# ZeningLin/PEneo

Measured on AMD Instinct MI355X. Metric: docs/sec fwd+bwd, LayoutLMv3-base seq512 L128, higher is better.
Workload: dtype bf16; 1 GPU; LayoutLMv3-base PEneo, synthetic RFUND-shaped batch seq512/128 lines, 8 docs/GPU, train mode (dropout 0.1), fwd+loss+bwd; docs_per_gpu=8, seq_len=512, lines=128, parallelism=dp1

## Files before the change

include/peneo_hip.h:

```cpp
#ifndef PENEO_HIP_H
#define PENEO_HIP_H

#include <stddef.h>
#include <stdint.h>

#ifdef __cplusplus
extern "C" {
#endif

#define PENEO_OK 0
#define PENEO_ERR_INVALID (-1)
#define PENEO_ERR_LAUNCH (-2)

#define PENEO_F32 0
#define PENEO_BF16 1

#define PENEO_ACT_NONE 0
#define PENEO_ACT_GELU 1
#define PENEO_ACT_SILU 2

#define PENEO_MAX_HEADS 8

typedef void* peneo_stream_t;

// ... 308 lines not shown
  int32_t step_offset; int32_t reserved;
} peneo_adamw_tensor;
int peneo_adamw_chunk_elems(void);
int peneo_adamw_step(const peneo_adamw_tensor* table_dev, const int32_t* chunk_tensor_dev, const int32_t* chunk_index_dev,
                     int n_chunks, float beta1, float beta2, float eps, int step, peneo_stream_t stream);
int peneo_grad_sqnorm_slots(void);
int peneo_grad_sqnorm(const peneo_adamw_tensor* table_dev, const int32_t* chunk_tensor_dev, const int32_t* chunk_index_dev,
                      int n_chunks, double* sqnorm_dev, peneo_stream_t stream);
int peneo_adamw_step_clip(const peneo_adamw_tensor* table_dev, const int32_t* chunk_tensor_dev, const int32_t* chunk_index_dev,
                          int n_chunks, float beta1, float beta2, float eps, int step, const double* sqnorm_dev,
                          float max_grad_norm, peneo_stream_t stream);
typedef struct peneo_adamw_emit { void* dst; int32_t tensor; int32_t dtype; } peneo_adamw_emit;
int peneo_adamw_step_emit(const peneo_adamw_tensor* table_dev, const int32_t* chunk_tensor_dev, const int32_t* chunk_index_dev,
                          int n_chunks, float beta1, float beta2, float eps, int step, const double* sqnorm_dev,
                          float max_grad_norm, const peneo_adamw_emit* emits_dev, const int32_t* emit_first_dev,
                          peneo_stream_t stream);

typedef struct peneo_encoder_layer {
  const void* Wqkv; const float* bqkv; const void* Wo; const float* bo; const float* g1; const float* b1;
  const void* Wi; const float* bi; const void* Wo2; const float* bo2; const float* g2; const float* b2;
  const void* bias; int64_t bias_ld; const float* key_bias; const uint32_t* drop_words;
  const void* x; void* qkv; void* att; float* lse; void* h1; float* m1; float* r1; void* a; void* zi; void* inter; void* h2;
  float* m2; float* r2;
  int32_t B, T, H, nh, I, reserved;
  float eps, attn_scale, p_hidden, p_attn;
  uint32_t seed_o, seed_o2;
} peneo_encoder_layer;
typedef struct peneo_encoder_layer_grads {
  const void* d_out; void* d_x;
  void* d_h2; void* d_dense2; void* d_zi; void* d_a; void* d_h1; void* d_dense1; void* d_att; void* dqkv; float* delta; void* ds_out;
  float* dwqkv; float* dbqkv; float* dwo; float* dbo; float* dg1; float* db1; float* dwi; float* dbi; float* dwo2; float* dbo2;
  float* dg2; float* db2;
} peneo_encoder_layer_grads;
size_t peneo_struct_bytes(int which);
size_t peneo_encoder_layer_workspace_bytes(int rows, int H, int I, int which);
int peneo_encoder_layer_fwd(const peneo_encoder_layer* layer, void* out, void* workspace, size_t workspace_bytes,
                            peneo_stream_t stream);
int peneo_encoder_layer_fwd_packed(const peneo_encoder_layer* layer, const int32_t* lens, const int32_t* cu_rows, int rows, void* out,
                                   void* workspace, size_t workspace_bytes, peneo_stream_t stream);
typedef struct peneo_encoder_layer_mxfp8 {
  const void* Wqkv_q; const void* Wqkv_s; const void* Wo_q; const void* Wo_s;
  const void* Wi_q; const void* Wi_s; const void* Wo2_q; const void* Wo2_s;
  void* x_q; void* x_s; void* att_q; void* att_s; void* a_q; void* a_s; void* inter_q; void* inter_s;
  void* out_q; void* out_s;
  int32_t x_prequantized, reserved;
} peneo_encoder_layer_mxfp8;
int peneo_encoder_layer_mxfp8_supported(int rows, int H, int I);
// ... 3 lines not shown
                            size_t ws_main_bytes, void* ws_side, size_t ws_side_bytes, peneo_stream_t stream,
                            peneo_stream_t side_stream);

int peneo_spots_to_tags(const int32_t* spots_bijt, int n_spots, int B, int N, int64_t* tags, int32_t* status,
                        peneo_stream_t stream);
int peneo_spots_compact(const float* logits, int64_t P, int C, int N, int32_t* spots_ijt, float* scores,
                        int32_t* count, int max_spots, peneo_stream_t stream);

typedef struct peneo_spots_batch_desc {
  int num_maps;
  int classes[PENEO_MAX_HEADS];
  const void* maps[PENEO_MAX_HEADS];
} peneo_spots_batch_desc;
size_t peneo_spots_compact_batch_workspace_bytes(int num_maps, int B, int N);
int peneo_spots_compact_batch(const peneo_spots_batch_desc* desc, int B, int N, void* records, int32_t* counts,
                              int max_spots, void* workspace, size_t workspace_bytes, peneo_stream_t stream);

void peneo_gemm_set_big_mode(int mode);
int peneo_gemm_big_mode(void);
void peneo_gemm_set_nn384_mode(int mode);
int peneo_gemm_nn384_mode(void);
uint64_t peneo_gemm_nn384_launches(void);
int peneo_gemm_nn384_shape_ok(int M, int N, int K);
void peneo_gemm_set_sk_mode(int mode);
void peneo_gemm_sk_set_prof(void* stamps);
void peneo_gemm_sk_set_max_groups(int n);

void peneo_set_deterministic(int mode);
int peneo_deterministic(void);
uint64_t peneo_order_dependent_launches(void);
int64_t peneo_pair_bwd_workspace_rows(int B, int N);
int64_t peneo_pair_dz_fused_workspace_rows(int64_t npairs);
size_t peneo_relpos_bwd_workspace_bytes(int nh, int bins1, int bins2);
int peneo_relpos_bias_bwd_layers_ws(const void* ds, int L, int64_t layer_stride, const uint8_t* bk1_t, const uint8_t* bkx_t,
                                    const uint8_t* bky_t, float* dw1, int bins1, float* dwx, float* dwy, int bins2, float scale,
                                    int B, int nh, int T, int Tp, void* workspace, size_t workspace_bytes, peneo_stream_t stream);
int peneo_relpos_bias_bwd_ws(const float* g, int64_t ldg, const uint8_t* bk1, const uint8_t* bkx, const uint8_t* bky, float* dw1,
                             int bins1, float* dwx, float* dwy, int bins2, float scale, int B, int nh, int T, void* workspace,
                             size_t workspace_bytes, peneo_stream_t stream);
size_t peneo_grad_sqnorm_workspace_bytes(int n_chunks);
int peneo_grad_sqnorm_ws(const peneo_adamw_tensor* table_dev, const int32_t* chunk_tensor_dev, const int32_t* chunk_index_dev,
                         int n_chunks, double* sqnorm_dev, void* workspace, size_t workspace_bytes, peneo_stream_t stream);

#ifdef __cplusplus
}
#endif
// ... 2 lines not shown
```

peneo_amd/csrc/common.h:

```cpp
#pragma once
#include <hip/hip_runtime.h>
#include <stdint.h>
#include <cstdlib>

#include "../../include/peneo_hip.h"

namespace peneo {

typedef unsigned short bf16_t;
typedef __attribute__((ext_vector_type(8))) __bf16 bf16x8_t;
typedef __attribute__((ext_vector_type(16))) float f32x16_t;
typedef __attribute__((ext_vector_type(4))) float f32x4_t;

constexpr int kWave = 64;

void set_error(const char* fmt, ...);
int check_launch(const char* what);

int det_mode();
int order_dependent(const char* entry_point);
#define PENEO_ORDER_DEPENDENT(entry_point)                        \
  do {                                                            \
    const int od_rc_ = ::peneo::order_dependent(entry_point);     \
    if (od_rc_ != PENEO_OK) return od_rc_;                        \
  } while (0)

inline int dynamic_lds_error(const char* entry_point, size_t bytes) {
  set_error("%s: cannot raise dynamic LDS to %zu bytes", entry_point, bytes);
  return PENEO_ERR_LAUNCH;
}
template <typename KernelT>
inline int raise_dynamic_lds(KernelT kernel, size_t bytes, const char* entry_point) {
  const void* fn = reinterpret_cast<const void*>(kernel);
  if (hipFuncSetAttribute(fn, hipFuncAttributeMaxDynamicSharedMemorySize, (int)bytes) == hipSuccess) return PENEO_OK;
  return dynamic_lds_error(entry_point, bytes);
}
inline bool env_switch_on(const char* name) { const char* e = getenv(name); return !e || atoi(e) != 0; }

#define PENEO_REQUIRE(cond, ...)                \
  do {                                          \
    if (!(cond)) {                              \
      ::peneo::set_error(__VA_ARGS__);          \
      return PENEO_ERR_INVALID;                 \
    }                                           \
  } while (0)

__device__ __forceinline__ float bf16_to_f32(bf16_t v) { return __uint_as_float(((uint32_t)v) << 16); }

// ... 273 lines not shown
```

peneo_amd/csrc/gemm.hip:

```cpp
#include <cstdlib>
#include "common.h"
#include "gemm_common.h"

namespace peneo {

__device__ __forceinline__ int lds_off(int row, int slot) { return row * ROWB + ((slot ^ ((row >> 1) & 7)) << 4); }

template <typename T> struct Stage { uint4 v[4]; };

template <typename T>
__device__ __forceinline__ uint4 guarded_vec_load(const T* base, int64_t ld, int r, int c, int rmax, int cmax) {
  constexpr int VEC = Elem<T>::kVec;
  uint4 z = make_uint4(0, 0, 0, 0);
  if (r >= rmax || c >= cmax) return z;
  const T* p = base + (int64_t)r * ld + c;
  if (c + VEC <= cmax && ((reinterpret_cast<uintptr_t>(p) & 15) == 0)) return *reinterpret_cast<const uint4*>(p);
  float f[VEC];
#pragma unroll
  for (int e = 0; e < VEC; ++e) f[e] = (c + e < cmax) ? Elem<T>::load(p + e) : 0.f;
  return pack16<T>(f);
}

template <typename T>
__device__ __forceinline__ void load_kmajor(Stage<T>& s, const T* base, int64_t ld, int r0, int k0, int rmax, int kmax,
// ... 672 lines not shown
  if constexpr (CS) {
    if (cs_on && (lane & 31) == 0) {
#pragma unroll
      for (int r = 0; r < 16; ++r) {
        const int m = m0 + wm * 64 + wn * 32 + acc_row(r, lane);
        if (m < p.M) atomicAdd(p.ep.a_colsum + m, accb[r]);
      }
    }
  }
  tile_epilogue<DZ>(p, acc, smem, m0, n0, tid, lane, wm, wn, dzpre, zsplit);
}

template <bool AK, bool BK, bool CS = false, bool DZ = false>
__global__ __launch_bounds__(256, 2) void gemm_dma_pipe_kernel(GemmParams p) {
  extern __shared__ __attribute__((aligned(16))) char smem[];
  const int gx = gridDim.x, gxy = gx * gridDim.y, total = gxy * gridDim.z;
  const int lin = (blockIdx.z * gridDim.y + blockIdx.y) * gx + blockIdx.x;
  const int q8 = total >> 3, r8 = total & 7, xcd = lin & 7, slot = lin >> 3;
  const int tile3 = xcd * q8 + min(xcd, r8) + slot;
  const int zsplit = tile3 / gxy, tile = tile3 - zsplit * gxy;
  gemm_dma_pipe_body<AK, BK, CS, DZ>(p, smem, (tile / gx) * GB, (tile % gx) * GB, zsplit, tile % gx, gx);
}

constexpr int GEMM_GROUP_MAX = 4;
struct GemmGroup {
  GemmParams p[GEMM_GROUP_MAX];
  int first_tile[GEMM_GROUP_MAX + 1];
  int gx[GEMM_GROUP_MAX];
  int n;
};
template <bool AK, bool BK>
__global__ __launch_bounds__(256, 2) void gemm_dma_pipe_group_kernel(GemmGroup g) {
  extern __shared__ __attribute__((aligned(16))) char smem[];
  const int total = gridDim.x, lin = blockIdx.x;
  const int q8 = total >> 3, r8 = total & 7, xcd = lin & 7, slot = lin >> 3;
  const int tile3 = xcd * q8 + min(xcd, r8) + slot;
  int i = 0;
#pragma unroll
  for (int k = 1; k < GEMM_GROUP_MAX; ++k)
    if (k < g.n && tile3 >= g.first_tile[k]) i = k;
  const int tile = tile3 - g.first_tile[i], gx = g.gx[i];
  gemm_dma_pipe_body<AK, BK>(g.p[i], smem, (tile / gx) * GB, (tile % gx) * GB, 0);
}

__global__ void splitk_reduce_kernel(GemmParams p) {
  int64_t idx = (int64_t)blockIdx.x * blockDim.x + threadIdx.x;
  int64_t total = (int64_t)p.M * p.N;
// ... 59 lines not shown
    return check_launch("peneo_gemm");
  }
  if (ak && bk) hipLaunchKernelGGL((gemm_dma_pipe_kernel<true, true>), grid, dim3(256), shmem, st, p);
  else if (ak && !bk) hipLaunchKernelGGL((gemm_dma_pipe_kernel<true, false>), grid, dim3(256), shmem, st, p);
  else if (!ak && bk) hipLaunchKernelGGL((gemm_dma_pipe_kernel<false, true>), grid, dim3(256), shmem, st, p);
  else if (p.ep.a_colsum) hipLaunchKernelGGL((gemm_dma_pipe_kernel<false, false, true>), grid, dim3(256), shmem, st, p);
  else hipLaunchKernelGGL((gemm_dma_pipe_kernel<false, false>), grid, dim3(256), shmem, st, p);
  return check_launch("peneo_gemm");
}


}

using namespace peneo;

extern "C" size_t peneo_gemm_workspace_bytes(int M, int N, int K, int split_k) {
  const size_t partials = split_k > 1 ? (size_t)split_k * (size_t)M * (size_t)N * sizeof(float) : 0;
  const size_t stream_k = gemm_sk_workspace_bytes(M, N, K);
  return partials > stream_k ? partials : stream_k;
}

extern "C" int peneo_gemm_group(int dtype, int a_kmajor, int b_kmajor, int c_dtype, const peneo_gemm_problem* problems, int n,
                                peneo_stream_t stream) {
  PENEO_REQUIRE(dtype == PENEO_BF16, "peneo_gemm_group: bf16 operands only");
  PENEO_REQUIRE(c_dtype == PENEO_F32 || c_dtype == PENEO_BF16, "peneo_gemm_group: bad c_dtype %d", c_dtype);
  PENEO_REQUIRE(problems && n >= 1 && n <= GEMM_GROUP_MAX, "peneo_gemm_group: 1..%d problems (got %d)", GEMM_GROUP_MAX, n);
  auto dma_ok = [](const void* ptr, int64_t ld, bool kmajor, int rows, int k) {
    return (reinterpret_cast<uintptr_t>(ptr) & 15) == 0 && (ld % 8) == 0 && ((kmajor ? k : rows) % 8) == 0 && rows >= 8;
  };
  GemmGroup g;
  g.n = n;
  int tiles = 0;
  for (int i = 0; i < GEMM_GROUP_MAX; ++i) {
    const peneo_gemm_problem& q = problems[i < n ? i : n - 1];
    if (i < n) {
      PENEO_REQUIRE(q.M > 0 && q.N > 0 && q.K > 0 && q.A && q.B && q.C, "peneo_gemm_group: problem %d is empty or has a null operand", i);
      PENEO_REQUIRE(q.lda >= (a_kmajor ? q.K : q.M) && q.ldb >= (b_kmajor ? q.K : q.N) && q.ldc >= q.N,
                    "peneo_gemm_group: problem %d: leading dim too small", i);
      PENEO_REQUIRE(dma_ok(q.A, q.lda, a_kmajor != 0, q.M, q.K) && dma_ok(q.B, q.ldb, b_kmajor != 0, q.N, q.K),
                    "peneo_gemm_group: problem %d: operands must be 16-byte aligned with extents in whole 16-byte chunks", i);
      PENEO_REQUIRE(!q.accumulate || c_dtype == PENEO_F32, "peneo_gemm_group: accumulate needs an fp32 C");
    }
    GemmParams& p = g.p[i];
    p.A = q.A; p.B = q.B; p.C = q.C; p.lda = q.lda; p.ldb = q.ldb; p.ldc = q.ldc; p.M = q.M; p.N = q.N; p.K = q.K;
    p.c_dtype = c_dtype;
    peneo_gemm_epilogue z = {};
    p.ep = (i < n && q.ep) ? *q.ep : z;
    if (i < n && q.ep) {
      PENEO_REQUIRE(!q.ep->pair_dz && !q.ep->a_colsum, "peneo_gemm_group: problem %d: pair_dz / a_colsum are not available in a group", i);
      PENEO_REQUIRE(q.ep->drop_p >= 0.f && q.ep->drop_p < 1.f, "peneo_gemm_group: problem %d: drop_p out of range", i);
      PENEO_REQUIRE(!q.ep->accumulate || c_dtype == PENEO_F32, "peneo_gemm_group: accumulate needs an fp32 C");
    }
    if (p.ep.alpha == 0.f) p.ep.alpha = 1.f;
    if (q.accumulate) p.ep.accumulate = 1;
    p.split_k = 1; p.ws = nullptr; p.kt_per_split = (q.K + 63) / 64; p.dz_on = 0; p.dz_ws = nullptr;
    peneo_pair_dz_args za = {};
    p.dz = za;
    g.first_tile[i] = tiles;
    g.gx[i] = (q.N + GB - 1) / GB;
    if (i < n) tiles += g.gx[i] * ((q.M + GB - 1) / GB);
  }
  g.first_tile[GEMM_GROUP_MAX] = tiles;
  for (int i = n; i < GEMM_GROUP_MAX; ++i) g.first_tile[i] = tiles;
  const int shmem = 2 * 2 * TILE_BYTES;
  hipStream_t st = reinterpret_cast<hipStream_t>(stream);
  const bool ak = a_kmajor != 0, bk = b_kmajor != 0;
#define PENEO_GROUP_LAUNCH(AK_, BK_)                                                                                         \
  {                                                                                                                          \
    static std::atomic<uint64_t> lds_devices{0};                                                                             \
    if (!allow_dynamic_lds(reinterpret_cast<const void*>(gemm_dma_pipe_group_kernel<AK_, BK_>), shmem, lds_devices))         \
      return dynamic_lds_error("peneo_gemm_group", shmem);                                                                   \
    hipLaunchKernelGGL((gemm_dma_pipe_group_kernel<AK_, BK_>), dim3((unsigned)tiles), dim3(256), shmem, st, g);              \
  }
  if (ak && bk) PENEO_GROUP_LAUNCH(true, true)
  else if (ak && !bk) PENEO_GROUP_LAUNCH(true, false)
  else if (!ak && bk) PENEO_GROUP_LAUNCH(false, true)
  else PENEO_GROUP_LAUNCH(false, false)
#undef PENEO_GROUP_LAUNCH
  return check_launch("peneo_gemm_group");
}

extern "C" int peneo_gemm(int dtype, int a_kmajor, int b_kmajor, int M, int N, int K, const void* A, int64_t lda,
                          const void* B, int64_t ldb, void* C, int64_t ldc, int c_dtype,
                          const peneo_gemm_epilogue* ep, int split_k, void* workspace, size_t workspace_bytes,
                          peneo_stream_t stream) {
  PENEO_REQUIRE(dtype == PENEO_F32 || dtype == PENEO_BF16, "peneo_gemm: bad dtype %d", dtype);
  PENEO_REQUIRE(c_dtype == PENEO_F32 || c_dtype == PENEO_BF16, "peneo_gemm: bad c_dtype %d", c_dtype);
  PENEO_REQUIRE(M > 0 && N > 0 && K > 0, "peneo_gemm: empty problem %dx%dx%d", M, N, K);
  PENEO_REQUIRE(A && B && C, "peneo_gemm: null operand");
// ... 86 lines not shown
```

peneo_amd/csrc/gemm_big.hip:

```cpp
#include <cstdlib>
#include <type_traits>
#include "common.h"
#include "gemm_common.h"

namespace peneo {

typedef short bg_s16x4 __attribute__((ext_vector_type(4)));

template <bool BK_, int WGM_, int WGN_, int FM_, int FN_, int NSTAGE_, bool AK_ = true>
struct BigCfg {
  static constexpr bool AK = AK_, BK = BK_;
  static constexpr int WGM = WGM_, WGN = WGN_, FM = FM_, FN = FN_, NSTAGE = NSTAGE_;
  static constexpr int BM = WGM * FM * 32, BN = WGN * FN * 32;
  static constexpr int A_BYTES = BM * 128, B_BYTES = BN * 128, STAGE = A_BYTES + B_BYTES;
  static constexpr int APW = BM / 64, BPW = BN / 64, PPW = APW + BPW;
  static constexpr int LDS_BYTES = NSTAGE * STAGE;
  static constexpr int EP_LD = FN * 32 + 4;
  static_assert(WGM * WGN == 8, "eight waves");
  static_assert(BM % 64 == 0 && BN % 64 == 0, "pieces of 8 rows are dealt to 8 waves");
  static_assert(8 * 32 * EP_LD * 4 <= LDS_BYTES, "epilogue patches fit in the dead ring");
  static_assert(LDS_BYTES <= 160 * 1024, "LDS");
};

template <typename C, bool PART = false>
__global__ __launch_bounds__(512) void gemm_big_kernel(GemmParams p, int tiles_n) {
  extern __shared__ __attribute__((aligned(16))) char smem[];
  constexpr int FM = C::FM, FN = C::FN, NSTAGE = C::NSTAGE;
  const int tid = threadIdx.x, lane = tid & 63, half = lane >> 5;
  const int wave = __builtin_amdgcn_readfirstlane(tid >> 6);
  const int wm = wave / C::WGN, wn = wave % C::WGN;

  const int total = gridDim.x, lin = blockIdx.x;
  const int q8 = total >> 3, r8 = total & 7, xcd = lin & 7, slot = lin >> 3;
  int tile = xcd * q8 + min(xcd, r8) + slot;
  int zsplit = 0, kt0 = 0, ktiles = p.K / 64;
  if constexpr (PART) {
    const int tiles = total / p.split_k;
    zsplit = tile / tiles;
    tile -= zsplit * tiles;
    kt0 = zsplit * p.kt_per_split;
    ktiles = min(ktiles, kt0 + p.kt_per_split) - kt0;
  }
  const int m0 = (tile / tiles_n) * C::BM, n0 = (tile % tiles_n) * C::BN;

  const bf16_t* A = reinterpret_cast<const bf16_t*>(p.A);
  const bf16_t* B = reinterpret_cast<const bf16_t*>(p.B);

  uint32_t offA[C::APW], offB[C::BPW];
#pragma unroll
  for (int u = 0; u < C::APW; ++u) {
    const int g = wave + 8 * u;
    if constexpr (C::AK) {
      const int row = g * 8 + (lane >> 3);
      const int sg = (lane & 7) ^ ((row >> 1) & 7);
      offA[u] = (uint32_t)(((int64_t)(min(m0 + row, p.M - 1) - m0) * p.lda + sg * 8) * 2);
    } else {
      constexpr int MQ = C::BM / 64;
      const int kb = g / MQ, mq = g % MQ, kr = lane >> 3;
      const int cg = (lane & 7) ^ (((kr >> 1) & 1) << 2);
      offA[u] = (uint32_t)(((int64_t)(kb * 8 + kr) * p.lda + (min(m0 + mq * 64 + cg * 8, p.M - 8) - m0)) * 2);
    }
  }
#pragma unroll
  for (int u = 0; u < C::BPW; ++u) {
    const int g = wave + 8 * u;
    if constexpr (C::BK) {
// ... 116 lines not shown
    const bool more = t + NSTAGE - 1 < ktiles;
    dbase = __builtin_amdgcn_readfirstlane(lds0 + ((t + NSTAGE - 1) % NSTAGE) * C::STAGE + wave * 1024);
    const char* st = smem + (t % NSTAGE) * C::STAGE;
    uint4 fa0[FM], fb0[FN], fa1[FM], fb1[FN];
    load_a(st, 0, fa0); load_b(st, 0, fb0);
    if (more) issue_group(std::integral_constant<int, 0>{});
    load_a(st, 1, fa1); load_b(st, 1, fb1);
    __builtin_amdgcn_sched_barrier(0);
    mma(fa0, fb0);
    __builtin_amdgcn_sched_barrier(0);
    if (more) issue_group(std::integral_constant<int, 1>{});
    load_a(st, 2, fa0); load_b(st, 2, fb0);
    __builtin_amdgcn_sched_barrier(0);
    mma(fa1, fb1);
    __builtin_amdgcn_sched_barrier(0);
    if (more) issue_group(std::integral_constant<int, 2>{});
    load_a(st, 3, fa1); load_b(st, 3, fb1);
    __builtin_amdgcn_sched_barrier(0);
    mma(fa0, fb0);
    __builtin_amdgcn_sched_barrier(0);
    if (more) issue_group(std::integral_constant<int, 3>{});
    mma(fa1, fb1);
  }
  __syncthreads();

  float* patch = reinterpret_cast<float*>(smem) + wave * (32 * C::EP_LD);
  constexpr int CG = FN * 32 / 8;
  constexpr int RPP = 64 / CG;
  constexpr int NPASS = (32 + RPP - 1) / RPP;
  const int cgi = lane % CG, rli = lane / CG;
  auto block = [&](auto ic) {
    constexpr int i = decltype(ic)::value;
#pragma unroll
    for (int j = 0; j < FN; ++j)
#pragma unroll
      for (int r = 0; r < 16; ++r) patch[acc_row(r, lane) * C::EP_LD + j * 32 + acc_col(lane)] = acc[i][j][r];
    __builtin_amdgcn_wave_barrier();
    const int mb = m0 + (wm * FM + i) * 32, nb = n0 + wn * FN * 32 + cgi * 8;
#pragma unroll 1
    for (int pass = 0; pass < NPASS; ++pass) {
      const int rl = pass * RPP + rli;
      if (rli < RPP && rl < 32 && mb + rl < p.M && nb + 8 <= p.N) {
        float v[8];
        const float4 x0 = *reinterpret_cast<const float4*>(patch + rl * C::EP_LD + cgi * 8);
        const float4 x1 = *reinterpret_cast<const float4*>(patch + rl * C::EP_LD + cgi * 8 + 4);
        v[0] = x0.x; v[1] = x0.y; v[2] = x0.z; v[3] = x0.w; v[4] = x1.x; v[5] = x1.y; v[6] = x1.z; v[7] = x1.w;
        if constexpr (PART) {
          float4* q = reinterpret_cast<float4*>(p.ws + ((int64_t)zsplit * p.M + (mb + rl)) * p.N + nb);
          q[0] = x0; q[1] = x1;
        } else {
          epilogue_store8(p, mb + rl, nb, v);
        }
      }
    }
    __builtin_amdgcn_wave_barrier();
  };
  block(std::integral_constant<int, 0>{});
  if constexpr (FM > 1) block(std::integral_constant<int, 1>{});
  if constexpr (FM > 2) block(std::integral_constant<int, 2>{});
  if constexpr (FM > 3) block(std::integral_constant<int, 3>{});
  static_assert(FM <= 4, "row blocks");
}

template <typename C, bool PART = false>
static int launch_big(const GemmParams& p, hipStream_t st) {
  const int tm = (p.M + C::BM - 1) / C::BM, tn = (p.N + C::BN - 1) / C::BN;
  static std::atomic<uint64_t> lds_devices{0};
  if (!allow_dynamic_lds(reinterpret_cast<const void*>(gemm_big_kernel<C, PART>), C::LDS_BYTES, lds_devices))
    return dynamic_lds_error("peneo_gemm", C::LDS_BYTES);
  const int wgs = tm * tn * (PART ? p.split_k : 1);
  hipLaunchKernelGGL((gemm_big_kernel<C, PART>), dim3((unsigned)wgs), dim3(512), C::LDS_BYTES, st, p, tn);
  const int rc = check_launch("peneo_gemm (big tiles)");
  return rc == PENEO_OK ? 1 : rc;
}

template <bool BK> using Big256 = BigCfg<BK, 2, 4, 4, 2, 2>;
template <bool BK> using Big384 = BigCfg<BK, 4, 2, 3, 3, 2>;
template <bool BK> using Big128 = BigCfg<BK, 4, 2, 2, 2, 3>;

static double big_cost(int M, int N, int bm, int bn, double per_round) {
  const int tiles = ((M + bm - 1) / bm) * ((N + bn - 1) / bn);
  return ((tiles + 255) / 256) * per_round;
}
static double small_cost(int M, int N) {
// ... 40 lines not shown
    if (pick == 128) return launch_big<Big128<true>>(p, st);
    return launch_big<Big256<true>>(p, st);
  }
  if (pick == 384) return launch_big<Big384<false>>(p, st);
  if (pick == 128) return launch_big<Big128<false>>(p, st);
  return launch_big<Big256<false>>(p, st);
}

using BigNN384 = BigCfg<false, 4, 2, 3, 3, 2, false>;
constexpr int NN_MIN_K = 65536;

static int g_nn_mode = -1;

static std::atomic<uint64_t> g_nn_launches{0};

static int nn_mode() {
  if (g_nn_mode < 0) { const char* e = getenv("PENEO_GEMM_NN384"); g_nn_mode = e ? atoi(e) : 1; }
  return big_mode() == 0 ? 0 : g_nn_mode;
}

static bool nn_shape_ok(int M, int N, int K) {
  const int mode = nn_mode();
  if (mode == 0 || M <= 0 || N <= 0 || K <= 0) return false;
  if (M % BigNN384::BM != 0 || N % BigNN384::BN != 0 || K % 64 != 0) return false;
  return mode != 1 || K >= NN_MIN_K;
}

int launch_gemm_big_nn(const GemmParams& p, hipStream_t st) {
  if (!nn_shape_ok(p.M, p.N, p.K)) return 0;
  const peneo_gemm_epilogue& e = p.ep;
  if (p.c_dtype != PENEO_F32 || p.dz_on || e.bias || e.preact || e.grad_src || e.residual || e.a_colsum || e.act != PENEO_ACT_NONE ||
      e.drop_p != 0.f || e.alpha != 1.f)
    return 0;
  if ((reinterpret_cast<uintptr_t>(p.A) | reinterpret_cast<uintptr_t>(p.B) | reinterpret_cast<uintptr_t>(p.C)) & 15) return 0;
  if (p.lda % 8 != 0 || p.ldb % 8 != 0 || p.ldc % 4 != 0) return 0;
  if ((int64_t)64 * p.lda * 2 >= ((int64_t)1 << 31) || (int64_t)64 * p.ldb * 2 >= ((int64_t)1 << 31)) return 0;
  if (p.split_k > 1 && (p.ws == nullptr || (reinterpret_cast<uintptr_t>(p.ws) & 15))) return 0;
  g_nn_launches.fetch_add(1, std::memory_order_relaxed);
  return p.split_k > 1 ? launch_big<BigNN384, true>(p, st) : launch_big<BigNN384, false>(p, st);
}

}

extern "C" void peneo_gemm_set_big_mode(int mode) { peneo::g_big_mode = mode; }
extern "C" int peneo_gemm_big_mode(void) { return peneo::big_mode(); }
extern "C" void peneo_gemm_set_nn384_mode(int mode) { peneo::g_nn_mode = mode; }
extern "C" int peneo_gemm_nn384_mode(void) { return peneo::nn_mode(); }
extern "C" int peneo_gemm_nn384_shape_ok(int M, int N, int K) { return peneo::nn_shape_ok(M, N, K) ? 1 : 0; }
extern "C" uint64_t peneo_gemm_nn384_launches(void) { return peneo::g_nn_launches.load(std::memory_order_relaxed); }
```

peneo_amd/csrc/gemm_common.h:

```cpp
#pragma once
#include <atomic>
#include "common.h"

namespace peneo {

constexpr int GB = 128;
constexpr int ROWB = 128;
constexpr int TILE_BYTES = GB * ROWB;

struct GemmParams {
  const void* A; const void* B; void* C;
  int64_t lda, ldb, ldc;
  int M, N, K;
  int c_dtype;
  peneo_gemm_epilogue ep;
  int split_k;
  float* ws;
  int kt_per_split;
  int dz_on;
  peneo_pair_dz_args dz;
  float* dz_ws;
};
constexpr int GEMM_DZ_SLOTS = 256;


__device__ __forceinline__ float load_any(const void* p, int dtype, int64_t idx) {
  return dtype == PENEO_F32 ? reinterpret_cast<const float*>(p)[idx] : bf16_to_f32(reinterpret_cast<const bf16_t*>(p)[idx]);
}
__device__ __forceinline__ void store_any(void* p, int dtype, int64_t idx, float v) {
  if (dtype == PENEO_F32) reinterpret_cast<float*>(p)[idx] = v;
  else reinterpret_cast<bf16_t*>(p)[idx] = f32_to_bf16(v);
}

__device__ __forceinline__ void epilogue_store(const GemmParams& p, int m, int n, float acc) {
  const peneo_gemm_epilogue& e = p.ep;
  float v = acc * e.alpha;
  if (e.bias) v += e.bias[n];
  if (e.preact) store_any(e.preact, p.c_dtype, (int64_t)m * e.ld_preact + n, v);
  const bool fast = p.c_dtype == PENEO_BF16;
  v = (fast && e.act == PENEO_ACT_GELU) ? gelu_fast_f(v) : act_f(e.act, v);
  if (e.grad_src) {
    const float g = load_any(e.grad_src, p.c_dtype, (int64_t)m * e.ld_grad + n);
    v *= (fast && e.grad_act == PENEO_ACT_GELU) ? gelu_grad_fast_f(g) : act_grad_f(e.grad_act, g);
  }
  if (e.drop_p > 0.f) {
// ... 163 lines not shown
  const int64_t ci = (int64_t)m * p.ldc + n;
  if (e.accumulate) {
    float c[8];
    load8_any(p.C, PENEO_F32, ci, c);
#pragma unroll
    for (int i = 0; i < 8; ++i) v[i] += c[i];
  }
  store8_any(p.C, p.c_dtype, ci, v);
}


inline bool allow_dynamic_lds(const void* kernel, int bytes, std::atomic<uint64_t>& devices) {
  int dev = 0;
  if (hipGetDevice(&dev) != hipSuccess) return false;
  const uint64_t bit = dev >= 0 && dev < 64 ? uint64_t(1) << dev : 0;
  if (devices.load(std::memory_order_acquire) & bit) return true;
  if (hipFuncSetAttribute(kernel, hipFuncAttributeMaxDynamicSharedMemorySize, bytes) != hipSuccess) return false;
  devices.fetch_or(bit, std::memory_order_release);
  return true;
}

int launch_gemm_big(const GemmParams& p, bool b_kmajor, hipStream_t st);
int launch_gemm_big_nn(const GemmParams& p, hipStream_t st);
int launch_gemm_sk(const GemmParams& p, bool b_kmajor, void* ws, size_t ws_bytes, hipStream_t st);
size_t gemm_sk_workspace_bytes(int M, int N, int K);

}
```

peneo_amd/csrc/stages.hip:

```cpp
#include <cstdlib>
#include <mutex>
#include "common.h"

using namespace peneo;

namespace {

int auto_split(int M, int N, int K) {
  const int tiles = ((M + 127) / 128) * ((N + 127) / 128);
  const int kt = (K + 63) / 64;
  if (tiles >= 192 || kt < 8) return 1;
  int s = kt / 4;
  if (512 / tiles < s) s = 512 / tiles;
  if (s > 16) s = 16;
  return s < 1 ? 1 : s;
}
size_t ws_bytes(int M, int N, int K) { return peneo_gemm_workspace_bytes(M, N, K, auto_split(M, N, K)); }
size_t max2(size_t a, size_t b) { return a > b ? a : b; }

struct Ws { void* p; size_t n; };
int gemm(int ak, int bk, int M, int N, int K, const void* A, int64_t lda, const void* B, int64_t ldb, void* C, int64_t ldc,
         int c_dtype, const peneo_gemm_epilogue& ep, Ws ws, hipStream_t st) {
  return peneo_gemm(PENEO_BF16, ak, bk, M, N, K, A, lda, B, ldb, C, ldc, c_dtype, &ep, auto_split(M, N, K), ws.p, ws.n, st);
}
// ... 199 lines not shown
  STAGE_TRY(peneo_colsum(PENEO_BF16, d_dense2, H, R, H, G->dbo2, 1, side));
  if (!grouped) STAGE_TRY(gemm(0, 0, H, I, R, d_dense2, H, L->inter, I, G->dwo2, I, PENEO_F32, ep, wsd, side));
  STAGE_TRY(peneo_colsum(PENEO_BF16, G->d_zi, I, R, I, G->dbi, 1, side));
  if (!grouped) STAGE_TRY(gemm(0, 0, I, H, R, G->d_zi, I, L->a, H, G->dwi, H, PENEO_F32, ep, wsd, side));
  STAGE_TRY(peneo_colsum(PENEO_BF16, d_dense1, H, R, H, G->dbo, 1, side));
  if (!grouped) STAGE_TRY(gemm(0, 0, H, H, R, d_dense1, H, L->att, H, G->dwo, H, PENEO_F32, ep, wsd, side));
  const char* qkv = reinterpret_cast<const char*>(L->qkv);
  char* dqkv = reinterpret_cast<char*>(G->dqkv);
  STAGE_TRY(peneo_attn_bwd(PENEO_BF16, qkv, qkv + 2 * (size_t)H, qkv + 4 * (size_t)H, 3 * H, nullptr, nullptr, nullptr, L->att, G->d_att, H, L->lse,
                           L->B, L->nh, L->T, d, L->attn_scale, L->bias, L->bias_ld, L->key_bias, dqkv, dqkv + 2 * (size_t)H, dqkv + 4 * (size_t)H,
                           3 * H, nullptr, G->delta, nullptr, G->ds_out, L->p_attn, L->p_attn > 0.f ? L->drop_words : nullptr, main));
  if (ev) {
    if (hipEventRecord(ev->e[1], main) != hipSuccess || hipStreamWaitEvent(side, ev->e[1], 0) != hipSuccess) return check_launch("peneo_encoder_layer_bwd (event)");
  }
  STAGE_TRY(peneo_colsum(PENEO_BF16, G->dqkv, 3 * H, R, 3 * H, G->dbqkv, 1, side));
  if (!grouped) {
    STAGE_TRY(gemm(0, 0, 3 * H, H, R, G->dqkv, 3 * H, L->x, H, G->dwqkv, H, PENEO_F32, ep, wsd, side));
  } else {
    peneo_gemm_problem pr[4] = {};
    pr[0] = {3 * H, H, R, G->dqkv, 3 * H, L->x, H, G->dwqkv, H, 0, nullptr};
    pr[1] = {I, H, R, G->d_zi, I, L->a, H, G->dwi, H, 0, nullptr};
    pr[2] = {H, I, R, d_dense2, H, L->inter, I, G->dwo2, I, 0, nullptr};
    pr[3] = {H, H, R, d_dense1, H, L->att, H, G->dwo, H, 0, nullptr};
    STAGE_TRY(peneo_gemm_group(PENEO_BF16, 0, 0, PENEO_F32, pr, 4, side));
  }
  ep = {};
  ep.residual = G->d_h1; ep.ld_res = H;
  STAGE_TRY(gemm(1, 0, R, H, 3 * H, G->dqkv, 3 * H, L->Wqkv, H, G->d_x, H, PENEO_BF16, ep, wm, main));
  return PENEO_OK;
}
```

peneo_amd/hip.py:

```python
from __future__ import annotations

import ctypes as C
import os
from typing import Optional, Sequence

import torch

_HERE = os.path.dirname(os.path.abspath(__file__))
LIB_PATH = os.environ.get("PENEO_HIP_LIB") or os.path.join(_HERE, "lib", "libpeneo_hip.so")

F32, BF16 = 0, 1
ACT_NONE, ACT_GELU, ACT_SILU = 0, 1, 2
MAX_HEADS = 8

_vp, _i, _i64, _f, _u32, _sz = C.c_void_p, C.c_int, C.c_int64, C.c_float, C.c_uint32, C.c_size_t


class PeneoHipError(RuntimeError):
    pass


class GemmEpilogue(C.Structure):
    _fields_ = [
        ("bias", _vp), ("act", _i), ("preact", _vp), ("ld_preact", _i64),
        ("grad_src", _vp), ("ld_grad", _i64), ("grad_act", _i),
        ("residual", _vp), ("ld_res", _i64), ("alpha", _f), ("accumulate", _i),
        ("drop_p", _f), ("drop_seed", _u32), ("pair_dz", _vp), ("pair_dz_ws", _vp), ("a_colsum", _vp),
    ]


class EncoderLayer(C.Structure):
    _fields_ = ([(n, _vp) for n in ("Wqkv", "bqkv", "Wo", "bo", "g1", "b1", "Wi", "bi", "Wo2", "bo2", "g2", "b2", "bias")] +
                [("bias_ld", _i64)] +
                [(n, _vp) for n in ("key_bias", "drop_words", "x", "qkv", "att", "lse", "h1", "m1", "r1", "a", "zi", "inter", "h2",
                                    "m2", "r2")] +
                [(n, _i) for n in ("B", "T", "H", "nh", "I", "reserved")] +
                [(n, _f) for n in ("eps", "attn_scale", "p_hidden", "p_attn")] + [("seed_o", _u32), ("seed_o2", _u32)])


class EncoderLayerMxfp8(C.Structure):
    _fields_ = [(n, _vp) for n in ("Wqkv_q", "Wqkv_s", "Wo_q", "Wo_s", "Wi_q", "Wi_s", "Wo2_q", "Wo2_s",
                                   "x_q", "x_s", "att_q", "att_s", "a_q", "a_s", "inter_q", "inter_s", "out_q", "out_s")] + \
               [("x_prequantized", _i), ("reserved", _i)]


class EncoderLayerGrads(C.Structure):
    _fields_ = [(n, _vp) for n in ("d_out", "d_x", "d_h2", "d_dense2", "d_zi", "d_a", "d_h1", "d_dense1", "d_att", "dqkv", "delta",
                                   "ds_out", "dwqkv", "dbqkv", "dwo", "dbo", "dg1", "db1", "dwi", "dbi", "dwo2", "dbo2", "dg2", "db2")]


class GemmProblem(C.Structure):
    _fields_ = [("M", _i), ("N", _i), ("K", _i), ("A", _vp), ("lda", _i64), ("B", _vp), ("ldb", _i64), ("C", _vp), ("ldc", _i64),
                ("accumulate", _i), ("ep", _vp)]


class CastItem(C.Structure):
    _fields_ = [("src", _vp), ("dst", _vp), ("numel", _i64)]


# ... 142 lines not shown
    "peneo_adamw_chunk_elems": (_i, []),
    "peneo_adamw_step": (_i, [_vp, _vp, _vp, _i, _f, _f, _f, _i, _vp]),
    "peneo_grad_sqnorm": (_i, [_vp, _vp, _vp, _i, _vp, _vp]),
    "peneo_grad_sqnorm_slots": (_i, []),
    "peneo_adamw_step_clip": (_i, [_vp, _vp, _vp, _i, _f, _f, _f, _i, _vp, _f, _vp]),
    "peneo_adamw_step_emit": (_i, [_vp, _vp, _vp, _i, _f, _f, _f, _i, _vp, _f, _vp, _vp, _vp]),
    "peneo_struct_bytes": (C.c_size_t, [_i]),
    "peneo_encoder_layer_workspace_bytes": (C.c_size_t, [_i, _i, _i, _i]),
    "peneo_encoder_layer_fwd": (_i, [_vp, _vp, _vp, C.c_size_t, _vp]),
    "peneo_encoder_layer_fwd_packed": (_i, [_vp, _vp, _vp, _i, _vp, _vp, C.c_size_t, _vp]),
    "peneo_encoder_layer_mxfp8_supported": (_i, [_i, _i, _i]),
    "peneo_encoder_layer_fwd_mxfp8": (_i, [_vp, _vp, _vp, _vp]),
    "peneo_encoder_layer_bwd": (_i, [_vp, _vp, _vp, C.c_size_t, _vp, C.c_size_t, _vp, _vp]),
    "peneo_spots_to_tags": (_i, [_vp, _i, _i, _i, _vp, _vp, _vp]),
    "peneo_spots_compact": (_i, [_vp, _i64, _i, _i, _vp, _vp, _vp, _i, _vp]),
    "peneo_spots_compact_batch_workspace_bytes": (_sz, [_i, _i, _i]),
    "peneo_spots_compact_batch": (_i, [C.POINTER(SpotsBatchDesc), _i, _i, _vp, _vp, _i, _vp, _sz, _vp]),
    "peneo_gemm_set_big_mode": (None, [_i]),
    "peneo_gemm_set_nn384_mode": (None, [_i]),
    "peneo_gemm_nn384_mode": (_i, []),
    "peneo_gemm_nn384_shape_ok": (_i, [_i, _i, _i]),
    "peneo_gemm_big_mode": (_i, []),
    "peneo_gemm_nn384_launches": (C.c_uint64, []),
    "peneo_gemm_set_sk_mode": (None, [_i]),
    "peneo_gemm_sk_set_prof": (None, [_vp]),
    "peneo_gemm_sk_set_max_groups": (None, [_i]),
    "peneo_set_deterministic": (None, [_i]),
    "peneo_deterministic": (_i, []),
    "peneo_order_dependent_launches": (C.c_uint64, []),
    "peneo_pair_bwd_workspace_rows": (_i64, [_i, _i]),
    "peneo_pair_dz_fused_workspace_rows": (_i64, [_i64]),
    "peneo_relpos_bwd_workspace_bytes": (_sz, [_i, _i, _i]),
    "peneo_relpos_bias_bwd_layers_ws": (_i, [_vp, _i, _i64, _vp, _vp, _vp, _vp, _i, _vp, _vp, _i, _f, _i, _i, _i, _i, _vp, _sz, _vp]),
    "peneo_relpos_bias_bwd_ws": (_i, [_vp, _i64, _vp, _vp, _vp, _vp, _i, _vp, _vp, _i, _f, _i, _i, _i, _vp, _sz, _vp]),
    "peneo_grad_sqnorm_workspace_bytes": (_sz, [_i]),
    "peneo_grad_sqnorm_ws": (_i, [_vp, _vp, _vp, _i, _vp, _vp, _sz, _vp]),
}

_lib: Optional[C.CDLL] = None


def load_library() -> C.CDLL:
    global _lib
    if _lib is not None:
        return _lib
    if not os.path.exists(LIB_PATH):
# ... 93 lines not shown
```

peneo_amd/model/modeling_layoutlmv3.py:

```python
from __future__ import annotations

import math
import os
from typing import List, Optional

import torch
import torch.nn as nn

import ctypes as C

from .. import ops
from ..hip import ACT_GELU, ACT_NONE, EncoderLayer, EncoderLayerGrads, EncoderLayerMxfp8, PeneoHipError, check, ptr
from ..hip import lib as hip_lib
from ..hip import stream as hip_stream
from .configuration_peneo import LayoutLMv3Config
from .engine import DropoutSeeds, can_defer, WeightCache, defer_join, join_pending, zeros_like_param, zeros_like_params
from .engine import side_stream as engine_side_stream
from .relpos import bucket_lut, visual_xy


class _SelfAttentionParams(nn.Module):
    def __init__(self, hidden: int):
        super().__init__()
        self.query = nn.Linear(hidden, hidden)
# ... 306 lines not shown
    L, keep = _describe_layer(model, st, idx, params, x, bufs)
    out = torch.empty((R, H), dtype=st.dtype, device=dev)
    wsb = _layer_ws_bytes(R, H, I, 0)
    ws = torch.empty(wsb, dtype=torch.uint8, device=dev) if wsb else None
    check(hip_lib().peneo_encoder_layer_fwd(C.byref(L), out.data_ptr(), ptr(ws), wsb, hip_stream()), "peneo_encoder_layer_fwd")
    ctx.model, ctx.st, ctx.idx = model, st, idx
    ctx.saved = (x, bufs)
    ctx.params = params
    ctx.stage_call = True
    return out


def _stage_backward(ctx, d_out):
    model, st, idx = ctx.model, ctx.st, ctx.idx
    params = ctx.params
    x, bufs = ctx.saved
    cfg, dt = model.config, st.dtype
    B, S, T = st.dims
    H, nh, I = cfg.hidden_size, cfg.num_attention_heads, cfg.intermediate_size
    R, dev = B * T, x.device
    seeds = st.seeds
    d_out = d_out.contiguous()
    L, keep = _describe_layer(model, st, idx, params, x, bufs)
    main = torch.cuda.current_stream()
    side = model.side_stream(dev) if model.wgrad_on_side_stream else None
    psz = 4 * H + (H + I + H + 3 * H)
    nl = len(model.encoder.layer)
    if getattr(st, "grad_pools", None) is None or idx == nl - 1:
        st.grad_pools = torch.zeros((nl, psz), dtype=torch.float32, device=dev)
    pool = st.grad_pools[idx]
    dg2, db2, dg1, db1 = pool[:H], pool[H:2 * H], pool[2 * H:3 * H], pool[3 * H:4 * H]
    o_ = 4 * H
    dbo2, dbi, dbo, dbqkv = pool[o_:o_ + H], pool[o_ + H:o_ + H + I], pool[o_ + H + I:o_ + 2 * H + I], pool[o_ + 2 * H + I:]
    if st.bias is not None and model.rel_tables_need_grad():
        if st.ds_layers is None:
            st.ds_layers = torch.empty((cfg.num_hidden_layers, B, nh, T, st.bias.shape[-1]), dtype=dt, device=dev)
        ds = st.ds_layers[idx]
    else:
        ds = torch.empty((B, nh, T, ops.attn_padded_len(T)), dtype=dt, device=dev)
    drop = seeds.p_hidden > 0
    nsc = R * (4 * H + (2 * H if drop else 0) + I + 3 * H)
    scratch = torch.empty(nsc, dtype=dt, device=dev)
    delta = torch.empty(B * nh * T, dtype=torch.float32, device=dev)
    d_x = torch.empty((R, H), dtype=dt, device=dev)
    dwqkv = torch.empty((3 * H, H), dtype=torch.float32, device=dev)
    dwo = torch.empty((H, H), dtype=torch.float32, device=dev)
# ... 512 lines not shown
```

Baseline: 526.0 docs/s.

## Route grouped weight-gradient GEMMs through the 384x192 big-tile kernel with K-tail support

```diff
diff --git a/include/peneo_hip.h b/include/peneo_hip.h
--- a/include/peneo_hip.h
+++ b/include/peneo_hip.h
@@ -354,7 +354,8 @@
   const void* bias; int64_t bias_ld; const float* key_bias; const uint32_t* drop_words;
   const void* x; void* qkv; void* att; float* lse; void* h1; float* m1; float* r1; void* a; void* zi; void* inter; void* h2;
   float* m2; float* r2;
-  int32_t B, T, H, nh, I, reserved;
+  int32_t B, T, H, nh, I;
+  int32_t wgrad_last;
   float eps, attn_scale, p_hidden, p_attn;
   uint32_t seed_o, seed_o2;
 } peneo_encoder_layer;
@@ -404,6 +405,9 @@
 int peneo_gemm_nn384_mode(void);
 uint64_t peneo_gemm_nn384_launches(void);
 int peneo_gemm_nn384_shape_ok(int M, int N, int K);
+void peneo_gemm_group_set_nn384_mode(int mode);
+int peneo_gemm_group_nn384_mode(void);
+uint64_t peneo_gemm_group_nn384_launches(void);
 void peneo_gemm_set_sk_mode(int mode);
 void peneo_gemm_sk_set_prof(void* stamps);
 void peneo_gemm_sk_set_max_groups(int n);
diff --git a/peneo_amd/csrc/common.h b/peneo_amd/csrc/common.h
--- a/peneo_amd/csrc/common.h
+++ b/peneo_amd/csrc/common.h
@@ -24,6 +24,10 @@
     const int od_rc_ = ::peneo::order_dependent(entry_point);     \
     if (od_rc_ != PENEO_OK) return od_rc_;                        \
   } while (0)
+
+int gemm_group_launch(int dtype, int a_kmajor, int b_kmajor, int c_dtype, const peneo_gemm_problem* problems, int n,
+                      peneo_stream_t stream, bool allow_nn384);
+int gemm_group_nn384_mode();
 
 inline int dynamic_lds_error(const char* entry_point, size_t bytes) {
   set_error("%s: cannot raise dynamic LDS to %zu bytes", entry_point, bytes);
diff --git a/peneo_amd/csrc/gemm.hip b/peneo_amd/csrc/gemm.hip
--- a/peneo_amd/csrc/gemm.hip
+++ b/peneo_amd/csrc/gemm.hip
@@ -718,7 +718,6 @@
   gemm_dma_pipe_body<AK, BK, CS, DZ>(p, smem, (tile / gx) * GB, (tile % gx) * GB, zsplit, tile % gx, gx);
 }
 
-constexpr int GEMM_GROUP_MAX = 4;
 struct GemmGroup {
   GemmParams p[GEMM_GROUP_MAX];
   int first_tile[GEMM_GROUP_MAX + 1];
@@ -824,6 +823,11 @@
 
 extern "C" int peneo_gemm_group(int dtype, int a_kmajor, int b_kmajor, int c_dtype, const peneo_gemm_problem* problems, int n,
                                 peneo_stream_t stream) {
+  return gemm_group_launch(dtype, a_kmajor, b_kmajor, c_dtype, problems, n, stream, true);
+}
+
+int peneo::gemm_group_launch(int dtype, int a_kmajor, int b_kmajor, int c_dtype, const peneo_gemm_problem* problems, int n,
+                             peneo_stream_t stream, bool allow_nn384) {
   PENEO_REQUIRE(dtype == PENEO_BF16, "peneo_gemm_group: bf16 operands only");
   PENEO_REQUIRE(c_dtype == PENEO_F32 || c_dtype == PENEO_BF16, "peneo_gemm_group: bad c_dtype %d", c_dtype);
   PENEO_REQUIRE(problems && n >= 1 && n <= GEMM_GROUP_MAX, "peneo_gemm_group: 1..%d problems (got %d)", GEMM_GROUP_MAX, n);
@@ -867,6 +871,10 @@
   const int shmem = 2 * 2 * TILE_BYTES;
   hipStream_t st = reinterpret_cast<hipStream_t>(stream);
   const bool ak = a_kmajor != 0, bk = b_kmajor != 0;
+  if (allow_nn384 && !ak && !bk && c_dtype == PENEO_F32) {
+    const int big = launch_gemm_big_group(g.p, n, st);
+    if (big != 0) return big < 0 ? big : PENEO_OK;
+  }
 #define PENEO_GROUP_LAUNCH(AK_, BK_)                                                                                         \
   {                                                                                                                          \
     static std::atomic<uint64_t> lds_devices{0};                                                                             \
diff --git a/peneo_amd/csrc/gemm_big.hip b/peneo_amd/csrc/gemm_big.hip
--- a/peneo_amd/csrc/gemm_big.hip
+++ b/peneo_amd/csrc/gemm_big.hip
@@ -2,6 +2,7 @@
 #include <type_traits>
 #include "common.h"
 #include "gemm_common.h"
+#include "gemm_walk.h"
 
 namespace peneo {
 
@@ -22,26 +23,27 @@
   static_assert(LDS_BYTES <= 160 * 1024, "LDS");
 };
 
-template <typename C, bool PART = false>
-__global__ __launch_bounds__(512) void gemm_big_kernel(GemmParams p, int tiles_n) {
-  extern __shared__ __attribute__((aligned(16))) char smem[];
+struct BigGroupProblem {
+  const void* A; const void* B; void* C;
+  int64_t lda, ldb, ldc;
+  int M, N, K, accumulate;
+};
+struct BigGroup {
+  BigGroupProblem q[GEMM_GROUP_MAX];
+  int first_tile[GEMM_GROUP_MAX + 1];
+  int tiles_n[GEMM_GROUP_MAX];
+  int n;
+};
+
+enum { EP_FUSED = 0, EP_PART = 1, EP_GROUP = 2 };
+
+template <typename C, int EPI, typename P>
+__device__ __forceinline__ void gemm_big_body(const P& p, char* smem, const int m0, const int n0, const int zsplit, const int kt0,
+                                              const int ktiles, const int tail_pieces) {
   constexpr int FM = C::FM, FN = C::FN, NSTAGE = C::NSTAGE;
   const int tid = threadIdx.x, lane = tid & 63, half = lane >> 5;
   const int wave = __builtin_amdgcn_readfirstlane(tid >> 6);
   const int wm = wave / C::WGN, wn = wave % C::WGN;
-
-  const int total = gridDim.x, lin = blockIdx.x;
-  const int q8 = total >> 3, r8 = total & 7, xcd = lin & 7, slot = lin >> 3;
-  int tile = xcd * q8 + min(xcd, r8) + slot;
-  int zsplit = 0, kt0 = 0, ktiles = p.K / 64;
-  if constexpr (PART) {
-    const int tiles = total / p.split_k;
-    zsplit = tile / tiles;
-    tile -= zsplit * tiles;
-    kt0 = zsplit * p.kt_per_split;
-    ktiles = min(ktiles, kt0 + p.kt_per_split) - kt0;
-  }
-  const int m0 = (tile / tiles_n) * C::BM, n0 = (tile % tiles_n) * C::BN;
 
   const bf16_t* A = reinterpret_cast<const bf16_t*>(p.A);
   const bf16_t* B = reinterpret_cast<const bf16_t*>(p.B);
@@ -204,6 +206,32 @@
     if (more) issue_group(std::integral_constant<int, 3>{});
     mma(fa1, fb1);
   }
+  if constexpr (!C::AK && !C::BK) {
+    static_assert(C::AK || C::BK || NSTAGE == 2, "the tail's vmcnt(0) argument above is the two-stage ring's");
+    if (tail_pieces > 0) {
+      __syncthreads();
+      dbase = __builtin_amdgcn_readfirstlane(lds0 + wave * 1024);
+      const uint4 zero4 = make_uint4(0u, 0u, 0u, 0u);
+#pragma unroll
+      for (int u = 0; u < C::APW; ++u) {
+        if (walk_piece_in_tail(wave + 8 * u, C::BM / 64, tail_pieces)) lds_dma_1k_s<0>(offA[u], bA, dbase + u * 8192);
+        else *reinterpret_cast<uint4*>(smem + (wave + 8 * u) * 1024 + lane * 16) = zero4;
+      }
+#pragma unroll
+      for (int u = 0; u < C::BPW; ++u) {
+        if (walk_piece_in_tail(wave + 8 * u, C::BN / 64, tail_pieces)) lds_dma_1k_s<0>(offB[u], bB, dbase + C::A_BYTES + u * 8192);
+        else *reinterpret_cast<uint4*>(smem + C::A_BYTES + (wave + 8 * u) * 1024 + lane * 16) = zero4;
+      }
+      wait_vm<0>();
+      __syncthreads();
+#pragma unroll
+      for (int ks = 0; ks < 4; ++ks) {
+        uint4 fa[FM], fb[FN];
+        load_a(smem, ks, fa); load_b(smem, ks, fb);
+        mma(fa, fb);
+      }
+    }
+  }
   __syncthreads();
 
   float* patch = reinterpret_cast<float*>(smem) + wave * (32 * C::EP_LD);
@@ -227,9 +255,16 @@
         const float4 x0 = *reinterpret_cast<const float4*>(patch + rl * C::EP_LD + cgi * 8);
         const float4 x1 = *reinterpret_cast<const float4*>(patch + rl * C::EP_LD + cgi * 8 + 4);
         v[0] = x0.x; v[1] = x0.y; v[2] = x0.z; v[3] = x0.w; v[4] = x1.x; v[5] = x1.y; v[6] = x1.z; v[7] = x1.w;
-        if constexpr (PART) {
+        if constexpr (EPI == EP_PART) {
           float4* q = reinterpret_cast<float4*>(p.ws + ((int64_t)zsplit * p.M + (mb + rl)) * p.N + nb);
           q[0] = x0; q[1] = x1;
+        } else if constexpr (EPI == EP_GROUP) {
+          float4* q = reinterpret_cast<float4*>(reinterpret_cast<float*>(p.C) + (int64_t)(mb + rl) * p.ldc + nb);
+          if (p.accumulate) {
+            const float4 c0 = q[0], c1 = q[1];
+            v[0] += c0.x; v[1] += c0.y; v[2] += c0.z; v[3] += c0.w; v[4] += c1.x; v[5] += c1.y; v[6] += c1.z; v[7] += c1.w;
+          }
+          q[0] = make_float4(v[0], v[1], v[2], v[3]); q[1] = make_float4(v[4], v[5], v[6], v[7]);
         } else {
           epilogue_store8(p, mb + rl, nb, v);
         }
@@ -242,6 +277,36 @@
   if constexpr (FM > 2) block(std::integral_constant<int, 2>{});
   if constexpr (FM > 3) block(std::integral_constant<int, 3>{});
   static_assert(FM <= 4, "row blocks");
+}
+
+template <typename C, bool PART = false>
+__global__ __launch_bounds__(512) void gemm_big_kernel(GemmParams p, int tiles_n) {
+  extern __shared__ __attribute__((aligned(16))) char smem[];
+  const int total = gridDim.x, lin = blockIdx.x;
+  const int q8 = total >> 3, r8 = total & 7, xcd = lin & 7, slot = lin >> 3;
+  int tile = xcd * q8 + min(xcd, r8) + slot;
+  constexpr bool TAIL = !C::AK && !C::BK;
+  const int kfull = p.K / 64;
+  int zsplit = 0, kt0 = 0, ktiles = kfull, tail = TAIL ? walk_tail_pieces(p.K) : 0;
+  if constexpr (PART) {
+    const int tiles = total / p.split_k;
+    zsplit = tile / tiles;
+    tile -= zsplit * tiles;
+    kt0 = zsplit * p.kt_per_split;
+    const int kend = kt0 + p.kt_per_split;
+    ktiles = min(kfull, kend) - kt0;
+    if (TAIL && kend <= kfull) tail = 0;
+  }
+  const int m0 = (tile / tiles_n) * C::BM, n0 = (tile % tiles_n) * C::BN;
+  gemm_big_body<C, PART ? EP_PART : EP_FUSED>(p, smem, m0, n0, zsplit, kt0, ktiles, tail);
+}
+
+template <typename C>
+__global__ __launch_bounds__(512) void gemm_big_group_kernel(BigGroup g) {
+  extern __shared__ __attribute__((aligned(16))) char smem[];
+  const WalkTile w = walk_group_tile(walk_xcd_tile(blockIdx.x, gridDim.x), g.first_tile, g.tiles_n, g.n, C::BM, C::BN);
+  const BigGroupProblem& q = g.q[w.problem];
+  gemm_big_body<C, EP_GROUP>(q, smem, w.m0, w.n0, 0, 0, q.K / 64, walk_tail_pieces(q.K));
 }
 
 template <typename C, bool PART = false>
@@ -328,7 +393,7 @@
 static bool nn_shape_ok(int M, int N, int K) {
   const int mode = nn_mode();
   if (mode == 0 || M <= 0 || N <= 0 || K <= 0) return false;
-  if (M % BigNN384::BM != 0 || N % BigNN384::BN != 0 || K % 64 != 0) return false;
+  if (M % BigNN384::BM != 0 || N % BigNN384::BN != 0 || K % 8 != 0) return false;
   return mode != 1 || K >= NN_MIN_K;
 }
 
@@ -346,6 +411,53 @@
   return p.split_k > 1 ? launch_big<BigNN384, true>(p, st) : launch_big<BigNN384, false>(p, st);
 }
 
+static int g_group_nn_mode = -1;
+static std::atomic<uint64_t> g_group_nn_launches{0};
+
+static int group_nn_mode() {
+  if (g_group_nn_mode < 0) {
+    const char* e = getenv("PENEO_WGRAD_NN384");
+    const int v = e ? atoi(e) : 1;
+    g_group_nn_mode = v < 0 ? 0 : v;
+  }
+  return big_mode() == 0 ? 0 : g_group_nn_mode;
+}
+
+int launch_gemm_big_group(const GemmParams* ps, int n, hipStream_t st) {
+  if (group_nn_mode() == 0 || n < 1 || n > GEMM_GROUP_MAX) return 0;
+  BigGroup g;
+  g.n = n;
+  int Ms[GEMM_GROUP_MAX], Ns[GEMM_GROUP_MAX];
+  for (int i = 0; i < GEMM_GROUP_MAX; ++i) {
+    const GemmParams& p = ps[i < n ? i : n - 1];
+    if (i < n) {
+      Ms[i] = p.M; Ns[i] = p.N;
+      const peneo_gemm_epilogue& e = p.ep;
+      if (p.c_dtype != PENEO_F32 || p.dz_on || p.split_k > 1 || e.bias || e.preact || e.grad_src || e.residual || e.a_colsum ||
+          e.act != PENEO_ACT_NONE || e.drop_p != 0.f || e.alpha != 1.f)
+        return 0;
+      if (p.M <= 0 || p.N <= 0 || p.K < 8 || p.M % BigNN384::BM != 0 || p.N % BigNN384::BN != 0 || p.K % 8 != 0) return 0;
+      if ((reinterpret_cast<uintptr_t>(p.A) | reinterpret_cast<uintptr_t>(p.B) | reinterpret_cast<uintptr_t>(p.C)) & 15) return 0;
+      if (p.lda % 8 != 0 || p.ldb % 8 != 0 || p.ldc % 4 != 0) return 0;
+      if ((int64_t)64 * p.lda * 2 >= ((int64_t)1 << 31) || (int64_t)64 * p.ldb * 2 >= ((int64_t)1 << 31)) return 0;
+    }
+    BigGroupProblem& q = g.q[i];
+    q.A = p.A; q.B = p.B; q.C = p.C; q.lda = p.lda; q.ldb = p.ldb; q.ldc = p.ldc; q.M = p.M; q.N = p.N; q.K = p.K;
+    q.accumulate = p.ep.accumulate ? 1 : 0;
+  }
+  const int tiles = walk_group_fill(Ms, Ns, n, GEMM_GROUP_MAX, BigNN384::BM, BigNN384::BN, g.first_tile, g.tiles_n);
+  static std::atomic<uint64_t> lds_devices{0};
+  if (!allow_dynamic_lds(reinterpret_cast<const void*>(gemm_big_group_kernel<BigNN384>), BigNN384::LDS_BYTES, lds_devices))
+    return dynamic_lds_error("peneo_gemm_group", BigNN384::LDS_BYTES);
+  hipLaunchKernelGGL((gemm_big_group_kernel<BigNN384>), dim3((unsigned)tiles), dim3(512), BigNN384::LDS_BYTES, st, g);
+  const int rc = check_launch("peneo_gemm_group (384 x 192 tiles)");
+  if (rc != PENEO_OK) return rc;
+  g_group_nn_launches.fetch_add(1, std::memory_order_relaxed);
+  return 1;
+}
+
+int gemm_group_nn384_mode() { return group_nn_mode(); }
+
 }
 
 extern "C" void peneo_gemm_set_big_mode(int mode) { peneo::g_big_mode = mode; }
@@ -354,3 +466,6 @@
 extern "C" int peneo_gemm_nn384_mode(void) { return peneo::nn_mode(); }
 extern "C" int peneo_gemm_nn384_shape_ok(int M, int N, int K) { return peneo::nn_shape_ok(M, N, K) ? 1 : 0; }
 extern "C" uint64_t peneo_gemm_nn384_launches(void) { return peneo::g_nn_launches.load(std::memory_order_relaxed); }
+extern "C" void peneo_gemm_group_set_nn384_mode(int mode) { peneo::g_group_nn_mode = mode < 0 ? 0 : mode; }
+extern "C" int peneo_gemm_group_nn384_mode(void) { return peneo::group_nn_mode(); }
+extern "C" uint64_t peneo_gemm_group_nn384_launches(void) { return peneo::g_group_nn_launches.load(std::memory_order_relaxed); }
diff --git a/peneo_amd/csrc/gemm_common.h b/peneo_amd/csrc/gemm_common.h
--- a/peneo_amd/csrc/gemm_common.h
+++ b/peneo_amd/csrc/gemm_common.h
@@ -21,6 +21,7 @@
   peneo_pair_dz_args dz;
   float* dz_ws;
 };
+constexpr int GEMM_GROUP_MAX = 4;
 constexpr int GEMM_DZ_SLOTS = 256;
 
 
@@ -230,6 +231,7 @@
 
 int launch_gemm_big(const GemmParams& p, bool b_kmajor, hipStream_t st);
 int launch_gemm_big_nn(const GemmParams& p, hipStream_t st);
+int launch_gemm_big_group(const GemmParams* ps, int n, hipStream_t st);
 int launch_gemm_sk(const GemmParams& p, bool b_kmajor, void* ws, size_t ws_bytes, hipStream_t st);
 size_t gemm_sk_workspace_bytes(int M, int N, int K);
 
diff --git a/peneo_amd/csrc/gemm_walk.h b/peneo_amd/csrc/gemm_walk.h
--- /dev/null
+++ b/peneo_amd/csrc/gemm_walk.h
@@ -0,0 +1,40 @@
+#pragma once
+
+#if defined(__HIPCC__)
+#define PENEO_WALK_FN __host__ __device__ inline
+#else
+#define PENEO_WALK_FN inline
+#endif
+
+namespace peneo {
+
+PENEO_WALK_FN int walk_xcd_tile(int lin, int total) {
+  const int q8 = total >> 3, r8 = total & 7, xcd = lin & 7, slot = lin >> 3;
+  return xcd * q8 + (xcd < r8 ? xcd : r8) + slot;
+}
+
+struct WalkTile { int problem, m0, n0; };
+PENEO_WALK_FN WalkTile walk_group_tile(int tile, const int* first_tile, const int* tiles_n, int n, int bm, int bn) {
+  int i = 0;
+  for (int k = 1; k < n; ++k)
+    if (tile >= first_tile[k]) i = k;
+  const int t = tile - first_tile[i];
+  return WalkTile{i, (t / tiles_n[i]) * bm, (t % tiles_n[i]) * bn};
+}
+
+PENEO_WALK_FN int walk_group_fill(const int* M, const int* N, int n, int max_n, int bm, int bn, int* first_tile, int* tiles_n) {
+  int tiles = 0;
+  for (int i = 0; i < max_n; ++i) {
+    const int j = i < n ? i : n - 1;
+    first_tile[i] = tiles;
+    tiles_n[i] = N[j] / bn;
+    if (i < n) tiles += (M[j] / bm) * (N[j] / bn);
+  }
+  first_tile[max_n] = tiles;
+  return tiles;
+}
+
+PENEO_WALK_FN int walk_tail_pieces(int K) { return ((K & 63) + 7) >> 3; }
+PENEO_WALK_FN bool walk_piece_in_tail(int g, int quads, int tail_pieces) { return g / quads < tail_pieces; }
+
+}
diff --git a/peneo_amd/csrc/stages.hip b/peneo_amd/csrc/stages.hip
--- a/peneo_amd/csrc/stages.hip
+++ b/peneo_amd/csrc/stages.hip
@@ -245,7 +245,8 @@
     pr[1] = {I, H, R, G->d_zi, I, L->a, H, G->dwi, H, 0, nullptr};
     pr[2] = {H, I, R, d_dense2, H, L->inter, I, G->dwo2, I, 0, nullptr};
     pr[3] = {H, H, R, d_dense1, H, L->att, H, G->dwo, H, 0, nullptr};
-    STAGE_TRY(peneo_gemm_group(PENEO_BF16, 0, 0, PENEO_F32, pr, 4, side));
+    const bool nn384 = !(gemm_group_nn384_mode() == 2 && L->wgrad_last);
+    STAGE_TRY(gemm_group_launch(PENEO_BF16, 0, 0, PENEO_F32, pr, 4, side, nn384));
   }
   ep = {};
   ep.residual = G->d_h1; ep.ld_res = H;
diff --git a/peneo_amd/hip.py b/peneo_amd/hip.py
--- a/peneo_amd/hip.py
+++ b/peneo_amd/hip.py
@@ -34,7 +34,7 @@
                 [("bias_ld", _i64)] +
                 [(n, _vp) for n in ("key_bias", "drop_words", "x", "qkv", "att", "lse", "h1", "m1", "r1", "a", "zi", "inter", "h2",
                                     "m2", "r2")] +
-                [(n, _i) for n in ("B", "T", "H", "nh", "I", "reserved")] +
+                [(n, _i) for n in ("B", "T", "H", "nh", "I", "wgrad_last")] +
                 [(n, _f) for n in ("eps", "attn_scale", "p_hidden", "p_attn")] + [("seed_o", _u32), ("seed_o2", _u32)])
 
 
@@ -223,6 +223,9 @@
     "peneo_gemm_nn384_shape_ok": (_i, [_i, _i, _i]),
     "peneo_gemm_big_mode": (_i, []),
     "peneo_gemm_nn384_launches": (C.c_uint64, []),
+    "peneo_gemm_group_set_nn384_mode": (None, [_i]),
+    "peneo_gemm_group_nn384_mode": (_i, []),
+    "peneo_gemm_group_nn384_launches": (C.c_uint64, []),
     "peneo_gemm_set_sk_mode": (None, [_i]),
     "peneo_gemm_sk_set_prof": (None, [_vp]),
     "peneo_gemm_sk_set_max_groups": (None, [_i]),
diff --git a/peneo_amd/model/modeling_layoutlmv3.py b/peneo_amd/model/modeling_layoutlmv3.py
--- a/peneo_amd/model/modeling_layoutlmv3.py
+++ b/peneo_amd/model/modeling_layoutlmv3.py
@@ -352,6 +352,7 @@
     seeds = st.seeds
     d_out = d_out.contiguous()
     L, keep = _describe_layer(model, st, idx, params, x, bufs)
+    L.wgrad_last = 1 if idx == 0 else 0
     main = torch.cuda.current_stream()
     side = model.side_stream(dev) if model.wgrad_on_side_stream else None
     psz = 4 * H + (H + I + H + 3 * H)
```

After: 536.8 docs/s (median of 6 runs). 2.0% higher.
